# JeongsooP/RGB-no-more

Hardware: AMD Instinct MI355X
Metric: images/sec JPEG-Ti DCT 512x512 train step (higher is better)
Workload: dtype bf16

## Files before the change

### rgb-no-more_amd/csrc/internal.h

```cpp
#pragma once
#include <hip/hip_runtime.h>

constexpr int RGBNM_TN_MAX_SPLIT = 128;
struct RgbnmTnJob {
  const void* dY; const void* X; float* part; float* bpart;
  int ldy, ldx, M, No, Ki;
  float* dW; float* db; int perm_heads, accumulate;
  int smax;
};
int rgbnm_launch_tn_pipe_group(const RgbnmTnJob* jobs, int n, int* S_out, hipStream_t st, int* direct_out = nullptr);
void rgbnm_tn_defer_begin();
void rgbnm_tn_defer_begin_n(int max_jobs);
int rgbnm_tn_defer_flush(hipStream_t st);
int rgbnm_launch_tn_pipe(const void* dY, int ldy, const void* X, int ldx, float* part, float* bpart, int M, int No,
                         int Ki, int* S_out, hipStream_t st, int smax = 0);

int rgbnm_launch_attn2_fwd(const void* qkv, void* out, float* lse, int B, int N, int heads, float scale,
                           hipStream_t st);
int rgbnm_launch_attn2_bwd(const void* qkv, const void* out, const void* dout, const float* lse, void* dqkv, int B,
                           int N, int heads, float scale, hipStream_t st);

enum { TR_NT = 1, TR_TN = 2, TR_ATTN_FWD = 3, TR_ATTN_BWD = 4, TR_CHAIN_FWD = 5, TR_CHAIN_BWD = 6, TR_AUG = 7, TR_EMBED = 8, TR_OPT = 9 };
int rgbnm_launch_nt_wres(int epi, const void* A, int lda, const void* W, int ldw, void* C, int ldc, const float* bias,
                         const void* R, int ldr, void* C2, int ldc2, int M, int N, int K, hipStream_t st);
int rgbnm_launch_nt_kpipe(int epi, const void* A, int lda, const void* W, int ldw, void* C, int ldc, const float* bias,
                          const void* R, int ldr, void* C2, int ldc2, int M, int N, int K, hipStream_t st);
int rgbnm_launch_nt_kpipe_res_ln(const void* A, int lda, const void* W, int ldw, const float* bias, const void* R,
                                 int ldr, void* x, int ldc, const float* gamma, const float* beta, void* y, int ldy,
                                 float* mean, float* rstd, float eps, int M, int N, int K, hipStream_t st);
int rgbnm_launch_mlp_fwd(const void* X, int ldx, const void* W1, const float* b1, const void* W2, const float* b2,
                         const void* R, int ldr, void* G, void* GP, int ldg, void* Y, int ldy, const float* gamma,
                         const float* beta, void* Y2, int ldy2, float* mean, float* rstd, float eps, int M, int E, int H,
                         hipStream_t st);
int rgbnm_launch_nt_small(int epi, const void* A, int lda, const void* W, int ldw, void* C, int ldc, const float* bias,
                          const void* R, int ldr, int c_f32, int M, int N, int K, hipStream_t st);
int rgbnm_launch_mlp_bwd(const void* DY, int lddy, const void* W2T, const void* W1T, const void* GP, int ldg, void* DU, int ldu,
                         const void* X, int ldx, const float* gamma, const float* mean, const float* rstd, void* DX, int lddx,
                         float* part, int* npanels_out, int M, int E, int H, hipStream_t st);
int rgbnm_launch_nt_kpipe_lnbwd(const void* A, int lda, const void* W, int ldw, const void* X, int ldx,
                                const float* gamma, const float* mean, const float* rstd, const void* dres, int ldr,
                                void* dx, int ldc, float* part, int* npanels_out, int M, int N, int K, hipStream_t st);
struct RgbnmReduceJob {
  const float* part; long long stride; float* out;
  int n, S, cols, perm_heads, accumulate, epw;
};
bool rgbnm_reduce_defer_active();
void rgbnm_reduce_defer_begin();
int rgbnm_reduce_defer_flush(hipStream_t st);
int rgbnm_reduce_submit(const RgbnmReduceJob& job, hipStream_t st);
int rgbnm_trace_begin(int tag, double flops, double bytes, hipStream_t st);
void rgbnm_trace_end(int slot, hipStream_t st);
```

### rgb-no-more_amd/csrc/layernorm.hip

```cpp
#include "common.h"
#include "../../include/rgbnm.h"
#include "internal.h"

namespace {


template <int LPR>
__device__ __forceinline__ float row_sum(float v) {
  if constexpr (LPR == 16) return group16_sum(v);
  else if constexpr (LPR == 32) return group16_sum(v + __shfl_xor(v, 16, 64));
  else return wave_sum(v);
}

template <typename T, int NV, int LPR = 16>
__global__ __launch_bounds__(256) void ln_fwd_kernel(const T* __restrict__ x, const float* __restrict__ gamma,
                                                     const float* __restrict__ beta, T* __restrict__ y,
                                                     float* __restrict__ mean, float* __restrict__ rstd, int M,
                                                     float eps) {
  constexpr int E = NV * LPR * 4, G = 256 / LPR;
  const int l16 = threadIdx.x & (LPR - 1), grp = threadIdx.x / LPR;
  f32x4 gm[NV], bt[NV];
#pragma unroll
  for (int v = 0; v < NV; ++v) {
    gm[v] = *reinterpret_cast<const f32x4*>(gamma + (v * LPR + l16) * 4);
    bt[v] = *reinterpret_cast<const f32x4*>(beta + (v * LPR + l16) * 4);
  }
  for (int row = blockIdx.x * G + grp; row < M; row += gridDim.x * G) {
#pragma clang fp contract(off)
    f32x4 xv[NV];
    float s = 0.f;
#pragma unroll
    for (int v = 0; v < NV; ++v) {
      xv[v] = load4<T>(x + (size_t)row * E + (v * LPR + l16) * 4);
      s += xv[v][0] + xv[v][1] + xv[v][2] + xv[v][3];
    }
// ... 91 lines not shown
      float a = 0.f;
#pragma unroll
      for (int r = 0; r < G; ++r) a += red[r][e];
      part[((size_t)blockIdx.x * 2 + pass) * E + e] = a;
    }
  }
}

int submit_ln_reduce(const float* part, float* dgamma, float* dbeta, int nblk, int E, int accumulate, hipStream_t st) {
  RgbnmReduceJob j;
  j.part = part; j.stride = 2LL * E; j.out = dgamma; j.n = E; j.S = nblk; j.cols = 1; j.perm_heads = 0;
  j.accumulate = accumulate; j.epw = 8;
  const bool own = !rgbnm_reduce_defer_active();
  if (own) rgbnm_reduce_defer_begin();
  int rc = rgbnm_reduce_submit(j, st);
  if (rc == RGBNM_OK) {
    j.part = part + E; j.out = dbeta;
    rc = rgbnm_reduce_submit(j, st);
  }
  if (own) {
    const int rf = rgbnm_reduce_defer_flush(st);
    if (rc == RGBNM_OK) rc = rf;
  }
  return rc;
}

template <typename T, int NV, int LPR = 16>
__global__ __launch_bounds__(256) void pool_fwd_kernel(const T* __restrict__ x, const float* __restrict__ gamma,
                                                       const float* __restrict__ beta, T* __restrict__ pooled,
                                                       float* __restrict__ mean, float* __restrict__ rstd, int N,
                                                       float eps) {
  constexpr int E = NV * LPR * 4, G = 256 / LPR;
  __shared__ float red[G][E + 4];
  const int b = blockIdx.x;
  const int l16 = threadIdx.x & (LPR - 1), grp = threadIdx.x / LPR;
  f32x4 acc[NV];
#pragma unroll
  for (int v = 0; v < NV; ++v) acc[v] = (f32x4){0.f, 0.f, 0.f, 0.f};
  constexpr int UNR = 8;
  for (int t0 = grp; t0 < N; t0 += UNR * G) {
    f32x4 xa[UNR][NV];
#pragma unroll
    for (int u = 0; u < UNR; ++u) {
      const int tt = min(t0 + u * G, N - 1);
#pragma unroll
      for (int v = 0; v < NV; ++v) xa[u][v] = load4<T>(x + ((size_t)b * N + tt) * E + (v * LPR + l16) * 4);
    }
#pragma unroll
    for (int u = 0; u < UNR; ++u) {
    const int t = t0 + u * G;
    if (t >= N) break;
    const size_t row = (size_t)b * N + t;
    f32x4 xv[NV];
    float s = 0.f;
#pragma unroll
    for (int v = 0; v < NV; ++v) {
      xv[v] = xa[u][v];
      s += xv[v][0] + xv[v][1] + xv[v][2] + xv[v][3];
    }
    const float mu = row_sum<LPR>(s) * (1.f / E);
    float q = 0.f;
#pragma unroll
    for (int v = 0; v < NV; ++v)
#pragma unroll
      for (int i = 0; i < 4; ++i) {
        const float d = xv[v][i] - mu;
        q += d * d;
      }
    const float rs = rsqrtf(row_sum<LPR>(q) * (1.f / E) + eps);
#pragma unroll
    for (int v = 0; v < NV; ++v)
#pragma unroll
      for (int i = 0; i < 4; ++i) acc[v][i] += (xv[v][i] - mu) * rs;
    if (l16 == 0) {
      mean[row] = mu;
      rstd[row] = rs;
    }
    }
  }
#pragma unroll
  for (int v = 0; v < NV; ++v)
#pragma unroll
    for (int i = 0; i < 4; ++i) red[grp][(v * LPR + l16) * 4 + i] = acc[v][i];
  __syncthreads();
  for (int e = threadIdx.x; e < E; e += 256) {
    float a = 0.f;
#pragma unroll
    for (int r = 0; r < G; ++r) a += red[r][e];
    pooled[(size_t)b * E + e] = from_f32<T>(a * (1.f / N) * gamma[e] + beta[e]);
  }
}

template <typename T, int NV, int LPR = 16>
__global__ __launch_bounds__(256) void pool_bwd_kernel(const T* __restrict__ dpooled, const T* __restrict__ x,
                                                       const float* __restrict__ gamma, const float* __restrict__ mean,
                                                       const float* __restrict__ rstd, T* __restrict__ dx,
                                                       float* __restrict__ part, int N) {
  constexpr int E = NV * LPR * 4, G = 256 / LPR;
  __shared__ float red[G][E + 4];
  const int b = blockIdx.x;
  const int l16 = threadIdx.x & (LPR - 1), grp = threadIdx.x / LPR;
  const float invN = 1.f / N;
  f32x4 gm[NV], dv[NV], dg[NV];
#pragma unroll
  for (int v = 0; v < NV; ++v) {
    gm[v] = *reinterpret_cast<const f32x4*>(gamma + (v * LPR + l16) * 4);
    dv[v] = load4<T>(dpooled + (size_t)b * E + (v * LPR + l16) * 4);
#pragma unroll
    for (int i = 0; i < 4; ++i) dv[v][i] *= invN;
    dg[v] = (f32x4){0.f, 0.f, 0.f, 0.f};
  }
  constexpr int UNR = 4;
  for (int t0 = grp; t0 < N; t0 += UNR * G) {
    f32x4 xa[UNR][NV];
    float mua[UNR], rsa[UNR];
#pragma unroll
    for (int u = 0; u < UNR; ++u) {
      const int tt = min(t0 + u * G, N - 1);
      mua[u] = mean[(size_t)b * N + tt];
      rsa[u] = rstd[(size_t)b * N + tt];
#pragma unroll
      for (int v = 0; v < NV; ++v) xa[u][v] = load4<T>(x + ((size_t)b * N + tt) * E + (v * LPR + l16) * 4);
    }
#pragma unroll
    for (int u = 0; u < UNR; ++u) {
    const int t = t0 + u * G;
    if (t >= N) break;
    const size_t row = (size_t)b * N + t;
    const float mu = mua[u], rs = rsa[u];
    f32x4 xh[NV], gv[NV];
    float s1 = 0.f, s2 = 0.f;
#pragma unroll
    for (int v = 0; v < NV; ++v) {
      const f32x4 xv = xa[u][v];
#pragma unroll
      for (int i = 0; i < 4; ++i) {
        xh[v][i] = (xv[i] - mu) * rs;
        gv[v][i] = dv[v][i] * gm[v][i];
        s1 += gv[v][i];
        s2 += gv[v][i] * xh[v][i];
        dg[v][i] += dv[v][i] * xh[v][i];
      }
    }
    const float c1 = row_sum<LPR>(s1) * (1.f / E), c2 = row_sum<LPR>(s2) * (1.f / E);
#pragma unroll
    for (int v = 0; v < NV; ++v) {
      f32x4 o;
#pragma unroll
      for (int i = 0; i < 4; ++i) o[i] = rs * (gv[v][i] - c1 - xh[v][i] * c2);
      store4<T>(dx + row * E + (v * LPR + l16) * 4, o);
    }
    }
  }
#pragma unroll
  for (int v = 0; v < NV; ++v)
#pragma unroll
    for (int i = 0; i < 4; ++i) red[grp][(v * LPR + l16) * 4 + i] = dg[v][i];
  __syncthreads();
  for (int e = threadIdx.x; e < E; e += 256) {
    float a = 0.f;
#pragma unroll
    for (int r = 0; r < G; ++r) a += red[r][e];
    part[((size_t)b * 2 + 0) * E + e] = a;
    part[((size_t)b * 2 + 1) * E + e] = to_f32(dpooled[(size_t)b * E + e]);
  }
}

constexpr int LN_BWD_BLOCKS = 2048;

template <typename T>
int ln_fwd_t(const void* x, const float* g, const float* b, void* y, float* mean, float* rstd, int M, int E, float eps,
             hipStream_t st) {
  const int grid = min(cdiv(M, E <= 384 ? 16 : 4), 4096);
  if (E == 192) hipLaunchKernelGGL((ln_fwd_kernel<T, 3>), dim3(grid), dim3(256), 0, st, (const T*)x, g, b, (T*)y, mean, rstd, M, eps);
  else if (E == 384) hipLaunchKernelGGL((ln_fwd_kernel<T, 6>), dim3(grid), dim3(256), 0, st, (const T*)x, g, b, (T*)y, mean, rstd, M, eps);
  else if (E == 512) hipLaunchKernelGGL((ln_fwd_kernel<T, 2, 64>), dim3(grid), dim3(256), 0, st, (const T*)x, g, b, (T*)y, mean, rstd, M, eps);
  else if (E == 768) hipLaunchKernelGGL((ln_fwd_kernel<T, 3, 64>), dim3(grid), dim3(256), 0, st, (const T*)x, g, b, (T*)y, mean, rstd, M, eps);
  else if (E == 1024) hipLaunchKernelGGL((ln_fwd_kernel<T, 4, 64>), dim3(grid), dim3(256), 0, st, (const T*)x, g, b, (T*)y, mean, rstd, M, eps);
  else return RGBNM_EINVAL;
  LAUNCH_CHECK();
  return RGBNM_OK;
}

template <typename T>
int ln_bwd_t(const void* dy, const void* x, const float* g, const float* mean, const float* rstd, const void* dres,
             void* dx, float* dgamma, float* dbeta, int M, int E, int accumulate, float* ws, hipStream_t st) {
  const int P = cdiv(M, E == 192 ? 16 : E == 384 ? 8 : 4), grid = cdiv(P, cdiv(P, LN_BWD_BLOCKS));
  if (E == 192) hipLaunchKernelGGL((ln_bwd_kernel<T, 3>), dim3(grid), dim3(256), 0, st, (const T*)dy, (const T*)x, g, mean, rstd, (const T*)dres, (T*)dx, ws, M);
  else if (E == 384) hipLaunchKernelGGL((ln_bwd_kernel<T, 3, 32>), dim3(grid), dim3(256), 0, st, (const T*)dy, (const T*)x, g, mean, rstd, (const T*)dres, (T*)dx, ws, M);
  else if (E == 512) hipLaunchKernelGGL((ln_bwd_kernel<T, 2, 64>), dim3(grid), dim3(256), 0, st, (const T*)dy, (const T*)x, g, mean, rstd, (const T*)dres, (T*)dx, ws, M);
  else if (E == 768) hipLaunchKernelGGL((ln_bwd_kernel<T, 3, 64>), dim3(grid), dim3(256), 0, st, (const T*)dy, (const T*)x, g, mean, rstd, (const T*)dres, (T*)dx, ws, M);
  else if (E == 1024) hipLaunchKernelGGL((ln_bwd_kernel<T, 4, 64>), dim3(grid), dim3(256), 0, st, (const T*)dy, (const T*)x, g, mean, rstd, (const T*)dres, (T*)dx, ws, M);
  else return RGBNM_EINVAL;
  LAUNCH_CHECK();
  return submit_ln_reduce(ws, dgamma, dbeta, grid, E, accumulate, st);
}

}
// ... 86 lines not shown
```

### rgb-no-more_amd/csrc/vit.hip

```cpp
#include "common.h"
#include "../../include/rgbnm.h"

#define TRY(x)                 \
  do {                         \
    int rc__ = (x);            \
    if (rc__ != 0) return rc__; \
  } while (0)

static inline size_t max_sz(size_t a, size_t b) { return a > b ? a : b; }

#include <string.h>
#include <atomic>
#include <mutex>
#include <vector>
#include "internal.h"
namespace {
std::mutex g_trace_mu;
struct TraceRec { hipEvent_t a, b; int tag; double flops, bytes; };
std::vector<TraceRec> g_recs;
std::vector<hipEvent_t> g_event_pool;
hipEvent_t take_event() {
  if (!g_event_pool.empty()) { hipEvent_t e = g_event_pool.back(); g_event_pool.pop_back(); return e; }
  hipEvent_t e = nullptr;
  if (hipEventCreate(&e) != hipSuccess) return nullptr;
  return e;
}
struct Opt { const char* name; std::atomic<int> value; };
Opt g_opts[] = {{"nt_staged", 1}, {"tn_tr", 1}, {"tn_pipe", 1}, {"attn_v2", 1}, {"nt_wres", 1}, {"nt_kpipe", 1}, {"attn_persist", 1}, {"ln_fuse", 1}, {"tn_group", 2}, {"trace", 0}, {"tn_wgs", 512}, {"mlp_fuse", 1}, {"nt_cold", 0}, {"mlp_bwd", 1}, {"nt_small", 1}, {"mlp_dmast", 1}, {"gelu_table", 1}, {"ln_rows", 1}, {"kp8", 1}, {"win_xcd", 1}, {"kp_persist", 1}, {"fwd_chain", 1}, {"bwd_chain", 1}, {"tn_direct", 1}, {"tn_pack", 1}, {"tn_wide", 1}};
}

int rgbnm_trace_begin(int tag, double flops, double bytes, hipStream_t st) {
  int mask = 0;
  for (auto& o : g_opts) if (!strcmp(o.name, "trace")) mask = o.value.load(std::memory_order_relaxed);
  if (!((mask >> tag) & 1)) return -1;
  std::lock_guard<std::mutex> lk(g_trace_mu);
  TraceRec r;
  r.a = take_event();
  r.b = take_event();
  if (!r.a || !r.b) return -1;
  r.tag = tag; r.flops = flops; r.bytes = bytes;
  (void)hipEventRecord(r.a, st);
  g_recs.push_back(r);
  return (int)g_recs.size() - 1;
}
void rgbnm_trace_end(int slot, hipStream_t st) {
  if (slot < 0) return;
  std::lock_guard<std::mutex> lk(g_trace_mu);
  if (slot >= 0 && slot < (int)g_recs.size()) (void)hipEventRecord(g_recs[slot].b, st);
}

extern "C" {

int rgbnm_abi_version(void) { return RGBNM_ABI_VERSION; }

int rgbnm_set_option(const char* name, int value) {
  for (auto& o : g_opts)
    if (name && !strcmp(o.name, name)) { o.value.store(value, std::memory_order_relaxed); return RGBNM_OK; }
  return RGBNM_EINVAL;
}
int rgbnm_get_option(const char* name) {
  for (auto& o : g_opts)
// ... 283 lines not shown
    }
    if (pe_dx0) TRY(rgbnm_gemm_tn(dt, pe_dx0, E, pe_feat, 384, pe_dw, pe_db, M, E, 384, 0, 0, pe_ws, pe_ws_bytes, st));
    if (group) { tn_open = false; TRY(rgbnm_tn_defer_flush((hipStream_t)st)); }
    for (int i = 0; i < n; ++i) {
      RgbnmReduceJob j;
      j.stride = 2LL * E; j.n = E; j.S = c->B; j.cols = 1; j.perm_heads = 0; j.accumulate = 0; j.epw = 8;
      j.part = part2[i]; j.out = g[i]->dln2_g;
      TRY(rgbnm_reduce_submit(j, (hipStream_t)st));
      j.part = part2[i] + E; j.out = g[i]->dln2_b;
      TRY(rgbnm_reduce_submit(j, (hipStream_t)st));
      j.part = part1[i]; j.out = g[i]->dln1_g;
      TRY(rgbnm_reduce_submit(j, (hipStream_t)st));
      j.part = part1[i] + E; j.out = g[i]->dln1_b;
      TRY(rgbnm_reduce_submit(j, (hipStream_t)st));
    }
    return RGBNM_OK;
  }();
  const int rt = tn_open ? rgbnm_tn_defer_flush((hipStream_t)st) : RGBNM_OK;
  const int rf = rgbnm_reduce_defer_flush((hipStream_t)st);
  return rc != RGBNM_OK ? rc : (rt != RGBNM_OK ? rt : rf);
}

int rgbnm_vit_block_bwd_dw(const rgbnm_vit_cfg* c, const rgbnm_block_acts* a, const rgbnm_block_grads* g,
                           const rgbnm_block_scratch* s, const void* dy, const float* part2, const float* part1, void* st) {
  return rgbnm_vit_blocks_bwd_dw(c, 1, &a, &g, &s, &dy, &part2, &part1, st);
}

int rgbnm_patch_embed_fwd_mix(const rgbnm_vit_cfg* c, int in_dtype, const void* y, const void* cbcr, const float* lam_dev,
                              const float* conv16, const void* wpe, const float* bpe, const float* pos, void* feat, void* x0, int Hb,
                              int Wb, void* st) {
  if (!c) return RGBNM_EINVAL;
  const int M = c->B * c->N;
  if ((Hb / 2) * (Wb / 2) != c->N) return RGBNM_EINVAL;
  TRY(rgbnm_subblock_embed_mix(in_dtype, c->dtype, y, cbcr, lam_dev, conv16, feat, c->B, Hb, Wb, 0, st));
  TRY(rgbnm_gemm_nt(c->dtype, RGBNM_EPI_POS, feat, 384, wpe, 384, x0, c->E, bpe, 0, 0, 0, 0, pos, c->N, M, c->E, 384,
                    0, st));
  return RGBNM_OK;
}

int rgbnm_patch_embed_fwd(const rgbnm_vit_cfg* c, int in_dtype, const void* y, const void* cbcr, const float* conv16,
                          const void* wpe, const float* bpe, const float* pos, void* feat, void* x0, int Hb, int Wb,
                          void* st) {
  return rgbnm_patch_embed_fwd_mix(c, in_dtype, y, cbcr, nullptr, conv16, wpe, bpe, pos, feat, x0, Hb, Wb, st);
}

int rgbnm_patch_embed_bwd(const rgbnm_vit_cfg* c, const void* dx0, const void* feat, float* dwpe, float* dbpe,
                          void* ws, size_t ws_bytes, void* st) {
  if (!c) return RGBNM_EINVAL;
  return rgbnm_gemm_tn(c->dtype, dx0, c->E, feat, 384, dwpe, dbpe, c->B * c->N, c->E, 384, 0, 0, ws, ws_bytes, st);
}

int rgbnm_head_fwd(const rgbnm_vit_cfg* c, const rgbnm_head_params* p, const rgbnm_head_acts* a, void* st) {
  if (!c || !p || !a) return RGBNM_EINVAL;
  const int dt = c->dtype, E = c->E, C = p->n_classes;
  TRY(rgbnm_head_pool_fwd(dt, a->x, p->ln_g, p->ln_b, a->pooled, a->mean, a->rstd, c->B, c->N, E, c->ln_eps, st));
  TRY(rgbnm_gemm_nt(dt, RGBNM_EPI_TANH, a->pooled, E, p->w1, E, a->h1, E, p->b1, 0, 0, 0, 0, 0, 0, c->B, E, E, 0, st));
  TRY(rgbnm_gemm_nt(dt, RGBNM_EPI_NONE, a->h1, E, p->w2, E, a->logits, C, p->b2, 0, 0, 0, 0, 0, 0, c->B, C, E, 1, st));
  return RGBNM_OK;
}

size_t rgbnm_head_bwd_workspace(const rgbnm_vit_cfg* c, int n_classes) {
  if (!c) return 0;
  return ((rgbnm_gemm_tn_workspace(c->B, n_classes, c->E) + 255) & ~(size_t)255) + ((rgbnm_gemm_tn_workspace(c->B, c->E, c->E) + 255) & ~(size_t)255) +
         (size_t)c->B * 2 * c->E * sizeof(float);
}

int rgbnm_head_bwd(const rgbnm_vit_cfg* c, const rgbnm_head_params* p, const rgbnm_head_acts* a,
                   const rgbnm_head_grads* g, const void* dlogits, void* da, void* dpooled, void* dx, void* ws,
                   size_t ws_bytes, void* st) {
  if (!c || !p || !a || !g || !dlogits || !da || !dpooled || !dx) return RGBNM_EINVAL;
  const int dt = c->dtype, E = c->E, C = p->n_classes, B = c->B;
  const size_t s1 = (rgbnm_gemm_tn_workspace(B, C, E) + 255) & ~(size_t)255, s2 = (rgbnm_gemm_tn_workspace(B, E, E) + 255) & ~(size_t)255;
  const size_t s3 = (size_t)B * 2 * E * sizeof(float);
  const bool apart = ws_bytes >= s1 + s2 + s3;
  char* w1 = (char*)ws;
  char* w2 = apart ? w1 + s1 : w1;
  char* w3 = apart ? w2 + s2 : w1;
  const size_t b1 = apart ? s1 : ws_bytes, b2 = apart ? s2 : ws_bytes, b3 = apart ? ws_bytes - s1 - s2 : ws_bytes;
  const bool grouped = apart && rgbnm_get_option("tn_group") != 0;
  if (grouped) rgbnm_tn_defer_begin();
  const int rc = [&]() -> int {
    TRY(rgbnm_gemm_tn(dt, dlogits, C, a->h1, E, g->dw2, g->db2, B, C, E, 0, 0, w1, b1, st));
    TRY(rgbnm_gemm_nt(dt, RGBNM_EPI_DTANH, dlogits, C, p->w2_t, C, da, E, 0, a->h1, E, 0, 0, 0, 0, B, E, C, 0, st));
    TRY(rgbnm_gemm_tn(dt, da, E, a->pooled, E, g->dw1, g->db1, B, E, E, 0, 0, w2, b2, st));
    return RGBNM_OK;
  }();
  const int rt = grouped ? rgbnm_tn_defer_flush((hipStream_t)st) : RGBNM_OK;
  if (rc != RGBNM_OK) return rc;
  if (rt != RGBNM_OK) return rt;
  TRY(rgbnm_gemm_nt(dt, RGBNM_EPI_NONE, da, E, p->w1_t, E, dpooled, E, 0, 0, 0, 0, 0, 0, 0, B, E, E, 0, st));
  TRY(rgbnm_head_pool_bwd(dt, dpooled, a->x, p->ln_g, a->mean, a->rstd, dx, g->dln_g, g->dln_b, B, c->N, E, 0, w3, b3, st));
  return RGBNM_OK;
}

}
```

Measured before the change: 65690.

## Fuse patch-embed and classifier head fwd/bwd into single per-image kernels

Adds a fused patch-embed kernel that combines the subblock embedding mix with the projection GEMM, bias and positional add. It also adds fused head forward (pool+LN, tanh matvec, logits) and backward (dlogits matvec, dtanh, dpooled matvec, pool LN backward) kernels, one block per image. The aim is to remove several small kernel launches and intermediate global round-trips for small-M GEMMs. The trade-off is that the per-image blocks do matvecs with low MMA utilisation and limited parallelism, and the new paths are gated on bf16 with E=192.

```diff
diff --git a/rgb-no-more_amd/csrc/head_fused.hip b/rgb-no-more_amd/csrc/head_fused.hip
--- /dev/null
+++ b/rgb-no-more_amd/csrc/head_fused.hip
@@ -0,0 +1,200 @@
+#include "common.h"
+#include "internal.h"
+#include "pool_rows.h"
+
+namespace {
+
+constexpr int E = 192, NV = 3, LPR = 16, G = 256 / LPR;
+constexpr int CH = 1024;
+
+struct HeadFwd {
+  const bf16* x; const float* ln_g; const float* ln_b; const bf16* w1; const float* b1; const bf16* w2; const float* b2;
+  bf16* pooled; float* mean; float* rstd; bf16* h1; float* logits;
+  int N, C; float eps;
+};
+struct HeadBwd {
+  const bf16* dlogits; const bf16* w2t; const bf16* w1t; const bf16* h1; const bf16* x; const float* ln_g;
+  const float* mean; const float* rstd;
+  bf16* da; bf16* dpooled; bf16* dx; float* part;
+  int N, C;
+};
+
+__device__ __forceinline__ bf16x8 kfrag(const bf16* row, int k, int K) {
+  const bf16x8 zero = {0, 0, 0, 0, 0, 0, 0, 0};
+  return k < K ? *reinterpret_cast<const bf16x8*>(row + k) : zero;
+}
+
+__device__ __forceinline__ void matvec192(const bf16* a, const bf16* __restrict__ W, int ldw, int K, float (*part)[CH], int w,
+                                          int lane) {
+  const int l31 = lane & 31, g = lane >> 5;
+  const int ksteps = (K + 15) / 16, per = (ksteps + 3) / 4;
+  const int s0 = w * per, s1 = min(s0 + per, ksteps);
+  f32x16 acc[6];
+#pragma unroll
+  for (int t = 0; t < 6; ++t)
+#pragma unroll
+    for (int r = 0; r < 16; ++r) acc[t][r] = 0.f;
+  const bf16* wrow = W + (size_t)l31 * ldw;
+  for (int s = s0; s < s1; s += 4) {
+    Frag<bf16> fa[4], fw[4][6];
+#pragma unroll
+    for (int u = 0; u < 4; ++u) {
+      const int k = 16 * (s + u < s1 ? s + u : s1 - 1) + 8 * g;
+      fa[u].v = kfrag(a, k, K);
+#pragma unroll
+      for (int t = 0; t < 6; ++t) fw[u][t].v = kfrag(wrow + (size_t)(32 * t) * ldw, k, K);
+    }
+#pragma unroll
+    for (int u = 0; u < 4; ++u)
+      if (s + u < s1) {
+#pragma unroll
+        for (int t = 0; t < 6; ++t) mma(acc[t], fw[u][t], fa[u]);
+      }
+  }
+  if (l31 == 0) {
+#pragma unroll
+    for (int t = 0; t < 6; ++t)
+#pragma unroll
+      for (int q = 0; q < 4; ++q) {
+        const f32x4 v = {acc[t][4 * q + 0], acc[t][4 * q + 1], acc[t][4 * q + 2], acc[t][4 * q + 3]};
+        *reinterpret_cast<f32x4*>(&part[w][32 * t + 8 * q + 4 * g]) = v;
+      }
+  }
+}
+
+__device__ __forceinline__ float sum4(float (*part)[CH], int n) {
+  float v = part[0][n];
+#pragma unroll
+  for (int k = 1; k < 4; ++k) v += part[k][n];
+  return v;
+}
+
+__global__ __launch_bounds__(256) void head_fwd_fused_kernel(HeadFwd p) {
+  __shared__ float red[G][E + 4];
+  __shared__ __attribute__((aligned(16))) float part[4][CH];
+  __shared__ __attribute__((aligned(16))) bf16 sp[E], sh[E];
+  const int b = blockIdx.x, tid = threadIdx.x, lane = tid & 63;
+  const int w = __builtin_amdgcn_readfirstlane(tid >> 6);
+  const int l31 = lane & 31, g = lane >> 5;
+  pool_fwd_image<bf16, NV, LPR>(p.x, p.ln_g, p.ln_b, p.pooled, p.mean, p.rstd, p.N, p.eps, b, red, sp);
+  __syncthreads();
+  matvec192(sp, p.w1, E, E, part, w, lane);
+  __syncthreads();
+  if (tid < E) {
+    float v = sum4(part, tid);
+    v += p.b1[tid];
+    float x = (float)(bf16)v;
+    x = tanhf(x);
+    const bf16 o = (bf16)x;
+    p.h1[(size_t)b * E + tid] = o;
+    sh[tid] = o;
+  }
+  __syncthreads();
+  Frag<bf16> fa[3];
+#pragma unroll
+  for (int u = 0; u < 3; ++u) fa[u].v = *reinterpret_cast<const bf16x8*>(&sh[16 * (3 * w + u) + 8 * g]);
+  for (int c0 = 0; c0 < p.C; c0 += CH) {
+    const int cn = min(CH, p.C - c0);
+    for (int n0 = 0; n0 < cn; n0 += 8 * 32) {
+      Frag<bf16> fw[8][3];
+#pragma unroll
+      for (int t = 0; t < 8; ++t) {
+        const bf16* wrow = p.w2 + (size_t)min(c0 + n0 + 32 * t + l31, p.C - 1) * E + 16 * 3 * w + 8 * g;
+#pragma unroll
+        for (int u = 0; u < 3; ++u) fw[t][u].v = *reinterpret_cast<const bf16x8*>(wrow + 16 * u);
+      }
+#pragma unroll
+      for (int t = 0; t < 8; ++t) {
+        f32x16 acc;
+#pragma unroll
+        for (int r = 0; r < 16; ++r) acc[r] = 0.f;
+#pragma unroll
+        for (int u = 0; u < 3; ++u) mma(acc, fw[t][u], fa[u]);
+        if (l31 == 0) {
+#pragma unroll
+          for (int q = 0; q < 4; ++q) {
+            const int n = n0 + 32 * t + 8 * q + 4 * g;
+            const f32x4 v = {acc[4 * q + 0], acc[4 * q + 1], acc[4 * q + 2], acc[4 * q + 3]};
+            if (n < cn) *reinterpret_cast<f32x4*>(&part[w][n]) = v;
+          }
+        }
+      }
+    }
+    __syncthreads();
+    for (int n = tid; n < cn; n += 256) {
+      float v = sum4(part, n);
+      if (p.b2) v += p.b2[c0 + n];
+      p.logits[(size_t)b * p.C + c0 + n] = v;
+    }
+    __syncthreads();
+  }
+}
+
+__global__ __launch_bounds__(256) void head_bwd_fused_kernel(HeadBwd p) {
+  __shared__ float red[G][E + 4];
+  __shared__ __attribute__((aligned(16))) float part[4][CH];
+  __shared__ __attribute__((aligned(16))) bf16 sda[E], sdp[E];
+  const int b = blockIdx.x, tid = threadIdx.x, lane = tid & 63;
+  const int w = __builtin_amdgcn_readfirstlane(tid >> 6);
+  matvec192(p.dlogits + (size_t)b * p.C, p.w2t, p.C, p.C, part, w, lane);
+  __syncthreads();
+  if (tid < E) {
+    const float v = sum4(part, tid);
+    float x = (float)(bf16)v;
+    const float h = (float)p.h1[(size_t)b * E + tid];
+    x *= (1.f - h * h);
+    const bf16 o = (bf16)x;
+    p.da[(size_t)b * E + tid] = o;
+    sda[tid] = o;
+  }
+  __syncthreads();
+  matvec192(sda, p.w1t, E, E, part, w, lane);
+  __syncthreads();
+  if (tid < E) {
+    const float v = sum4(part, tid);
+    const float x = (float)(bf16)v;
+    const bf16 o = (bf16)x;
+    p.dpooled[(size_t)b * E + tid] = o;
+    sdp[tid] = o;
+  }
+  __syncthreads();
+  pool_bwd_image<bf16, NV, LPR>(sdp, p.x, p.ln_g, p.mean, p.rstd, p.dx, p.part, p.N, b, red);
+}
+
+}
+
+int rgbnm_launch_head_fwd_fused(const void* x, const float* ln_g, const float* ln_b, const void* w1, const float* b1, const void* w2,
+                                const float* b2, void* pooled, float* mean, float* rstd, void* h1, float* logits, int B, int N, int C,
+                                float eps, hipStream_t st) {
+  if (!x || !ln_g || !ln_b || !w1 || !b1 || !w2 || !pooled || !mean || !rstd || !h1 || !logits || B <= 0 || N <= 0) return RGBNM_EINVAL;
+  if (B > 512 || C <= 0 || C % 8) return 1;
+  HeadFwd p;
+  p.x = (const bf16*)x; p.ln_g = ln_g; p.ln_b = ln_b; p.w1 = (const bf16*)w1; p.b1 = b1; p.w2 = (const bf16*)w2; p.b2 = b2;
+  p.pooled = (bf16*)pooled; p.mean = mean; p.rstd = rstd; p.h1 = (bf16*)h1; p.logits = logits; p.N = N; p.C = C; p.eps = eps;
+  const double Bd = B;
+  const int slot = rgbnm_trace_begin(TR_NT, 2.0 * Bd * E * E + 2.0 * Bd * C * E,
+                                     (Bd * E + (double)E * E) * 2.0 + Bd * E * 2.0 + (Bd * E + (double)C * E) * 2.0 + Bd * C * 4.0, st);
+  hipLaunchKernelGGL(head_fwd_fused_kernel, dim3(B), dim3(256), 0, st, p);
+  rgbnm_trace_end(slot, st);
+  LAUNCH_CHECK();
+  return RGBNM_OK;
+}
+
+int rgbnm_launch_head_bwd_fused(const void* dlogits, const void* w2t, const void* w1t, const void* h1, const void* x, const float* ln_g,
+                                const float* mean, const float* rstd, void* da, void* dpooled, void* dx, float* part, int B, int N,
+                                int C, hipStream_t st) {
+  if (!dlogits || !w2t || !w1t || !h1 || !x || !ln_g || !mean || !rstd || !da || !dpooled || !dx || !part || B <= 0 || N <= 0)
+    return RGBNM_EINVAL;
+  if (B > 512 || C <= 0 || C % 8) return 1;
+  HeadBwd p;
+  p.dlogits = (const bf16*)dlogits; p.w2t = (const bf16*)w2t; p.w1t = (const bf16*)w1t; p.h1 = (const bf16*)h1; p.x = (const bf16*)x;
+  p.ln_g = ln_g; p.mean = mean; p.rstd = rstd; p.da = (bf16*)da; p.dpooled = (bf16*)dpooled; p.dx = (bf16*)dx; p.part = part;
+  p.N = N; p.C = C;
+  const double Bd = B;
+  const int slot = rgbnm_trace_begin(TR_NT, 2.0 * Bd * E * C + 2.0 * Bd * E * E,
+                                     (Bd * C + (double)E * C) * 2.0 + Bd * E * 4.0 + (Bd * E + (double)E * E) * 2.0 + Bd * E * 2.0, st);
+  hipLaunchKernelGGL(head_bwd_fused_kernel, dim3(B), dim3(256), 0, st, p);
+  rgbnm_trace_end(slot, st);
+  LAUNCH_CHECK();
+  return RGBNM_OK;
+}
diff --git a/rgb-no-more_amd/csrc/internal.h b/rgb-no-more_amd/csrc/internal.h
--- a/rgb-no-more_amd/csrc/internal.h
+++ b/rgb-no-more_amd/csrc/internal.h
@@ -34,6 +34,15 @@
                          hipStream_t st);
 int rgbnm_launch_nt_small(int epi, const void* A, int lda, const void* W, int ldw, void* C, int ldc, const float* bias,
                           const void* R, int ldr, int c_f32, int M, int N, int K, hipStream_t st);
+int rgbnm_launch_patch_embed_fused(int in_dtype, const void* y, const void* cbcr, const float* lam_dev, const float* conv16,
+                                   const void* wpe, const float* bpe, const float* pos, void* feat, void* x0, int B, int Hb, int Wb,
+                                   hipStream_t st);
+int rgbnm_launch_head_fwd_fused(const void* x, const float* ln_g, const float* ln_b, const void* w1, const float* b1, const void* w2,
+                                const float* b2, void* pooled, float* mean, float* rstd, void* h1, float* logits, int B, int N, int C,
+                                float eps, hipStream_t st);
+int rgbnm_launch_head_bwd_fused(const void* dlogits, const void* w2t, const void* w1t, const void* h1, const void* x, const float* ln_g,
+                                const float* mean, const float* rstd, void* da, void* dpooled, void* dx, float* part, int B, int N,
+                                int C, hipStream_t st);
 int rgbnm_launch_mlp_bwd(const void* DY, int lddy, const void* W2T, const void* W1T, const void* GP, int ldg, void* DU, int ldu,
                          const void* X, int ldx, const float* gamma, const float* mean, const float* rstd, void* DX, int lddx,
                          float* part, int* npanels_out, int M, int E, int H, hipStream_t st);
diff --git a/rgb-no-more_amd/csrc/layernorm.hip b/rgb-no-more_amd/csrc/layernorm.hip
--- a/rgb-no-more_amd/csrc/layernorm.hip
+++ b/rgb-no-more_amd/csrc/layernorm.hip
@@ -1,6 +1,7 @@
 #include "common.h"
 #include "../../include/rgbnm.h"
 #include "internal.h"
+#include "pool_rows.h"
 
 namespace {
 
@@ -158,63 +159,7 @@
                                                        float eps) {
   constexpr int E = NV * LPR * 4, G = 256 / LPR;
   __shared__ float red[G][E + 4];
-  const int b = blockIdx.x;
-  const int l16 = threadIdx.x & (LPR - 1), grp = threadIdx.x / LPR;
-  f32x4 acc[NV];
-#pragma unroll
-  for (int v = 0; v < NV; ++v) acc[v] = (f32x4){0.f, 0.f, 0.f, 0.f};
-  constexpr int UNR = 8;
-  for (int t0 = grp; t0 < N; t0 += UNR * G) {
-    f32x4 xa[UNR][NV];
-#pragma unroll
-    for (int u = 0; u < UNR; ++u) {
-      const int tt = min(t0 + u * G, N - 1);
-#pragma unroll
-      for (int v = 0; v < NV; ++v) xa[u][v] = load4<T>(x + ((size_t)b * N + tt) * E + (v * LPR + l16) * 4);
-    }
-#pragma unroll
-    for (int u = 0; u < UNR; ++u) {
-    const int t = t0 + u * G;
-    if (t >= N) break;
-    const size_t row = (size_t)b * N + t;
-    f32x4 xv[NV];
-    float s = 0.f;
-#pragma unroll
-    for (int v = 0; v < NV; ++v) {
-      xv[v] = xa[u][v];
-      s += xv[v][0] + xv[v][1] + xv[v][2] + xv[v][3];
-    }
-    const float mu = row_sum<LPR>(s) * (1.f / E);
-    float q = 0.f;
-#pragma unroll
-    for (int v = 0; v < NV; ++v)
-#pragma unroll
-      for (int i = 0; i < 4; ++i) {
-        const float d = xv[v][i] - mu;
-        q += d * d;
-      }
-    const float rs = rsqrtf(row_sum<LPR>(q) * (1.f / E) + eps);
-#pragma unroll
-    for (int v = 0; v < NV; ++v)
-#pragma unroll
-      for (int i = 0; i < 4; ++i) acc[v][i] += (xv[v][i] - mu) * rs;
-    if (l16 == 0) {
-      mean[row] = mu;
-      rstd[row] = rs;
-    }
-    }
-  }
-#pragma unroll
-  for (int v = 0; v < NV; ++v)
-#pragma unroll
-    for (int i = 0; i < 4; ++i) red[grp][(v * LPR + l16) * 4 + i] = acc[v][i];
-  __syncthreads();
-  for (int e = threadIdx.x; e < E; e += 256) {
-    float a = 0.f;
-#pragma unroll
-    for (int r = 0; r < G; ++r) a += red[r][e];
-    pooled[(size_t)b * E + e] = from_f32<T>(a * (1.f / N) * gamma[e] + beta[e]);
-  }
+  pool_fwd_image<T, NV, LPR>(x, gamma, beta, pooled, mean, rstd, N, eps, blockIdx.x, red, nullptr);
 }
 
 template <typename T, int NV, int LPR = 16>
@@ -224,72 +169,7 @@
                                                        float* __restrict__ part, int N) {
   constexpr int E = NV * LPR * 4, G = 256 / LPR;
   __shared__ float red[G][E + 4];
-  const int b = blockIdx.x;
-  const int l16 = threadIdx.x & (LPR - 1), grp = threadIdx.x / LPR;
-  const float invN = 1.f / N;
-  f32x4 gm[NV], dv[NV], dg[NV];
-#pragma unroll
-  for (int v = 0; v < NV; ++v) {
-    gm[v] = *reinterpret_cast<const f32x4*>(gamma + (v * LPR + l16) * 4);
-    dv[v] = load4<T>(dpooled + (size_t)b * E + (v * LPR + l16) * 4);
-#pragma unroll
-    for (int i = 0; i < 4; ++i) dv[v][i] *= invN;
-    dg[v] = (f32x4){0.f, 0.f, 0.f, 0.f};
-  }
-  constexpr int UNR = 4;
-  for (int t0 = grp; t0 < N; t0 += UNR * G) {
-    f32x4 xa[UNR][NV];
-    float mua[UNR], rsa[UNR];
-#pragma unroll
-    for (int u = 0; u < UNR; ++u) {
-      const int tt = min(t0 + u * G, N - 1);
-      mua[u] = mean[(size_t)b * N + tt];
-      rsa[u] = rstd[(size_t)b * N + tt];
-#pragma unroll
-      for (int v = 0; v < NV; ++v) xa[u][v] = load4<T>(x + ((size_t)b * N + tt) * E + (v * LPR + l16) * 4);
-    }
-#pragma unroll
-    for (int u = 0; u < UNR; ++u) {
-    const int t = t0 + u * G;
-    if (t >= N) break;
-    const size_t row = (size_t)b * N + t;
-    const float mu = mua[u], rs = rsa[u];
-    f32x4 xh[NV], gv[NV];
-    float s1 = 0.f, s2 = 0.f;
-#pragma unroll
-    for (int v = 0; v < NV; ++v) {
-      const f32x4 xv = xa[u][v];
-#pragma unroll
-      for (int i = 0; i < 4; ++i) {
-        xh[v][i] = (xv[i] - mu) * rs;
-        gv[v][i] = dv[v][i] * gm[v][i];
-        s1 += gv[v][i];
-        s2 += gv[v][i] * xh[v][i];
-        dg[v][i] += dv[v][i] * xh[v][i];
-      }
-    }
-    const float c1 = row_sum<LPR>(s1) * (1.f / E), c2 = row_sum<LPR>(s2) * (1.f / E);
-#pragma unroll
-    for (int v = 0; v < NV; ++v) {
-      f32x4 o;
-#pragma unroll
-      for (int i = 0; i < 4; ++i) o[i] = rs * (gv[v][i] - c1 - xh[v][i] * c2);
-      store4<T>(dx + row * E + (v * LPR + l16) * 4, o);
-    }
-    }
-  }
-#pragma unroll
-  for (int v = 0; v < NV; ++v)
-#pragma unroll
-    for (int i = 0; i < 4; ++i) red[grp][(v * LPR + l16) * 4 + i] = dg[v][i];
-  __syncthreads();
-  for (int e = threadIdx.x; e < E; e += 256) {
-    float a = 0.f;
-#pragma unroll
-    for (int r = 0; r < G; ++r) a += red[r][e];
-    part[((size_t)b * 2 + 0) * E + e] = a;
-    part[((size_t)b * 2 + 1) * E + e] = to_f32(dpooled[(size_t)b * E + e]);
-  }
+  pool_bwd_image<T, NV, LPR>(dpooled + (size_t)blockIdx.x * E, x, gamma, mean, rstd, dx, part, N, blockIdx.x, red);
 }
 
 constexpr int LN_BWD_BLOCKS = 2048;
diff --git a/rgb-no-more_amd/csrc/patch_embed_fused.hip b/rgb-no-more_amd/csrc/patch_embed_fused.hip
--- /dev/null
+++ b/rgb-no-more_amd/csrc/patch_embed_fused.hip
@@ -0,0 +1,192 @@
+#include "common.h"
+#include "internal.h"
+
+namespace {
+
+constexpr int PR = 98;
+constexpr int KF = 384, EO = 192;
+constexpr int PITCH = KF * 2 + 16;
+constexpr int XS_BYTES = 4 * 16 * 17 * 4;
+constexpr int SMEM = PR * PITCH + XS_BYTES;
+constexpr int PF = 6;
+
+struct PeFused {
+  const void* y; const void* cbcr; const float* A; const float* lam; const bf16* W; const float* bias; const float* pos;
+  bf16* feat; bf16* x0;
+  int B, Hb, Wb, nh, ps;
+};
+
+__device__ __forceinline__ float mix2(float a, float c, float l0, float l1) { return fmaf(c, l1, a * l0); }
+
+template <typename TI>
+__global__ __launch_bounds__(256) __attribute__((amdgpu_waves_per_eu(2, 2))) void patch_embed_fused_kernel(PeFused p) {
+  extern __shared__ __attribute__((aligned(16))) unsigned char smem[];
+  unsigned char* As = smem;
+  float (*Xs)[16][17] = reinterpret_cast<float (*)[16][17]>(smem + PR * PITCH);
+  const int tid = threadIdx.x, lane = tid & 63;
+  const int w = __builtin_amdgcn_readfirstlane(tid >> 6);
+  const int img = blockIdx.x / p.nh, panel = blockIdx.x % p.nh;
+  const int ph_n = p.Hb / 2, pw_n = p.Wb / 2, npos = ph_n * pw_n;
+  const int t0 = panel * p.ps, nr = min(p.ps, npos - t0);
+  if (nr <= 0) return;
+  bf16* featp = p.feat + ((size_t)img * npos + t0) * KF;
+  {
+    const TI* y = reinterpret_cast<const TI*>(p.y);
+    const TI* cbcr = reinterpret_cast<const TI*>(p.cbcr);
+    const int g = lane >> 4, c = lane & 15;
+    float a1[4], a2[4];
+#pragma unroll
+    for (int kk = 0; kk < 4; ++kk) {
+      a1[kk] = p.A[c * 16 + 4 * kk + g];
+      a2[kk] = p.A[c * 16 + 4 * g + kk];
+    }
+    const int pdh = lane >> 5, pdw = (lane >> 4) & 1, l16 = lane & 15;
+    const int p1 = l16 >> 1, p2 = (l16 & 1) * 4;
+    const int e0 = lane * 2, cc = e0 >> 6, k = e0 & 63;
+    const bool mixed = p.lam != nullptr;
+    const float l0 = mixed ? p.lam[0] : 1.f, l1 = mixed ? p.lam[1] : 0.f;
+    const size_t ypi = (size_t)p.Hb * p.Wb * 64, cpi = (size_t)2 * npos * 64;
+    const int pb = img == 0 ? p.B - 1 : img - 1;
+    struct alignas(2 * sizeof(TI)) TI2 { TI a, b; };
+    struct Raw { typename Vec4<TI>::type v; TI2 c; };
+    auto fetch = [&](int pos, int b, Raw& r) {
+      const int ph = pos / pw_n, pw = pos % pw_n;
+      r.v = *reinterpret_cast<const typename Vec4<TI>::type*>(y + b * ypi + ((size_t)(2 * ph + pdh) * p.Wb + 2 * pw + pdw) * 64 + l16 * 4);
+      r.c = *reinterpret_cast<const TI2*>(cbcr + b * cpi + (((size_t)cc * ph_n + ph) * pw_n + pw) * 64 + k);
+    };
+    int fi = w;
+    Raw rq[PF] = {}, sq[PF] = {};
+    auto fetch_next = [&](Raw& r, Raw& s) {
+      if (fi < nr) {
+        fetch(t0 + fi, img, r);
+        if (mixed) fetch(t0 + fi, pb, s);
+      }
+      fi += 4;
+    };
+#pragma unroll
+    for (int u = 0; u < PF; ++u) fetch_next(rq[u], sq[u]);
+    for (int i = w; i < nr; i += 4) {
+      const Raw cur = rq[0], prev = sq[0];
+#pragma unroll
+      for (int u = 0; u + 1 < PF; ++u) {
+        rq[u] = rq[u + 1];
+        sq[u] = sq[u + 1];
+      }
+      fetch_next(rq[PF - 1], sq[PF - 1]);
+      f32x4 v = {to_f32(cur.v[0]), to_f32(cur.v[1]), to_f32(cur.v[2]), to_f32(cur.v[3])};
+      float c0 = to_f32(cur.c.a), c1 = to_f32(cur.c.b);
+      if (mixed) {
+#pragma unroll
+        for (int e = 0; e < 4; ++e) v[e] = to_f32(from_f32<TI>(mix2(v[e], to_f32(prev.v[e]), l0, l1)));
+        c0 = to_f32(from_f32<TI>(mix2(c0, to_f32(prev.c.a), l0, l1)));
+        c1 = to_f32(from_f32<TI>(mix2(c1, to_f32(prev.c.b), l0, l1)));
+      }
+#pragma unroll
+      for (int e = 0; e < 4; ++e) Xs[w][8 * pdh + p1][8 * pdw + p2 + e] = v[e];
+      asm volatile("s_waitcnt lgkmcnt(0)" ::: "memory");
+      f32x4 t = {0.f, 0.f, 0.f, 0.f};
+#pragma unroll
+      for (int kk = 0; kk < 4; ++kk) t = __builtin_amdgcn_mfma_f32_16x16x4f32(Xs[w][4 * kk + g][c], a1[kk], t, 0, 0, 0);
+      asm volatile("s_waitcnt lgkmcnt(0)" ::: "memory");
+      f32x4 z = {0.f, 0.f, 0.f, 0.f};
+#pragma unroll
+      for (int kk = 0; kk < 4; ++kk) z = __builtin_amdgcn_mfma_f32_16x16x4f32(a2[kk], t[kk], z, 0, 0, 0);
+      const bf16x4 zb = {from_f32<bf16>(z[0]), from_f32<bf16>(z[1]), from_f32<bf16>(z[2]), from_f32<bf16>(z[3])};
+      struct alignas(4) Pair { bf16 a, b; };
+      Pair pr;
+      pr.a = from_f32<bf16>(c0);
+      pr.b = from_f32<bf16>(c1);
+      bf16* dst = featp + (size_t)i * KF;
+      *reinterpret_cast<bf16x4*>(dst + c * 16 + 4 * g) = zb;
+      *reinterpret_cast<Pair*>(dst + 256 + e0) = pr;
+      bf16* lrow = reinterpret_cast<bf16*>(As + i * PITCH);
+      *reinterpret_cast<bf16x4*>(lrow + c * 16 + 4 * g) = zb;
+      *reinterpret_cast<Pair*>(lrow + 256 + e0) = pr;
+    }
+  }
+  __syncthreads();
+  if (32 * w >= nr) return;
+  const int l31 = lane & 31, g = lane >> 5;
+  const int tl = min(32 * w + l31, nr - 1);
+  const unsigned char* arow = As + tl * PITCH + 16 * g;
+  const bf16* wrow = p.W + (size_t)l31 * KF + 8 * g;
+  f32x16 acc[6];
+#pragma unroll
+  for (int t = 0; t < 6; ++t)
+#pragma unroll
+    for (int r = 0; r < 16; ++r) acc[t][r] = 0.f;
+  for (int ks = 0; ks < KF / 16; ks += 4) {
+    Frag<bf16> fa[4], fw[4][6];
+#pragma unroll
+    for (int u = 0; u < 4; ++u) {
+      fa[u].v = *reinterpret_cast<const bf16x8*>(arow + (ks + u) * 32);
+#pragma unroll
+      for (int t = 0; t < 6; ++t) fw[u][t].v = *reinterpret_cast<const bf16x8*>(wrow + (size_t)(32 * t) * KF + 16 * (ks + u));
+    }
+#pragma unroll
+    for (int u = 0; u < 4; ++u)
+#pragma unroll
+      for (int t = 0; t < 6; ++t) mma(acc[t], fw[u][t], fa[u]);
+  }
+  asm volatile("s_waitcnt lgkmcnt(0)" ::: "memory");
+  const float* posr = p.pos + (size_t)(t0 + tl) * EO;
+  const bool valid = 32 * w + l31 < nr;
+  bf16* srow = reinterpret_cast<bf16*>(As + (32 * w + l31) * PITCH);
+#pragma unroll
+  for (int t = 0; t < 6; ++t)
+#pragma unroll
+    for (int q = 0; q < 4; ++q) {
+      const int nl = 32 * t + 8 * q + 4 * g;
+      f32x4 v = {acc[t][4 * q + 0], acc[t][4 * q + 1], acc[t][4 * q + 2], acc[t][4 * q + 3]};
+      if (p.bias) {
+        const f32x4 bv = *reinterpret_cast<const f32x4*>(p.bias + nl);
+        v += bv;
+      }
+      const f32x4 pv = *reinterpret_cast<const f32x4*>(posr + nl);
+      v += pv;
+      if (valid) store4<bf16>(srow + nl, v);
+    }
+  asm volatile("s_waitcnt lgkmcnt(0)" ::: "memory");
+  bf16* x0p = p.x0 + ((size_t)img * npos + t0 + 32 * w) * EO;
+#pragma unroll
+  for (int it = 0; it < 32 * (EO / 8) / 64; ++it) {
+    const int idx = it * 64 + lane, row = idx / (EO / 8), vec = idx % (EO / 8);
+    if (32 * w + row < nr) {
+      const bf16x8 cv = *reinterpret_cast<const bf16x8*>(As + (32 * w + row) * PITCH + vec * 16);
+      *reinterpret_cast<bf16x8*>(x0p + (size_t)row * EO + vec * 8) = cv;
+    }
+  }
+}
+
+}
+
+int rgbnm_launch_patch_embed_fused(int in_dtype, const void* y, const void* cbcr, const float* lam_dev, const float* conv16,
+                                   const void* wpe, const float* bpe, const float* pos, void* feat, void* x0, int B, int Hb, int Wb,
+                                   hipStream_t st) {
+  if (!y || !cbcr || !conv16 || !wpe || !pos || !feat || !x0 || B <= 0 || Hb <= 0 || Wb <= 0 || (Hb & 1) || (Wb & 1)) return RGBNM_EINVAL;
+  if (in_dtype != DT_F32 && in_dtype != DT_BF16) return 1;
+  const int npos = (Hb / 2) * (Wb / 2);
+  const long long npatch = (long long)B * npos;
+  if (npatch * KF >= (1LL << 31)) return RGBNM_EINVAL;
+  PeFused p;
+  p.y = y; p.cbcr = cbcr; p.A = conv16; p.lam = lam_dev; p.W = (const bf16*)wpe; p.bias = bpe; p.pos = pos;
+  p.feat = (bf16*)feat; p.x0 = (bf16*)x0; p.B = B; p.Hb = Hb; p.Wb = Wb;
+  p.nh = cdiv(npos, PR);
+  p.ps = cdiv(npos, p.nh);
+  static DevOnce attr;
+  if (attr.need()) {
+    if (hipFuncSetAttribute((const void*)patch_embed_fused_kernel<float>, hipFuncAttributeMaxDynamicSharedMemorySize, SMEM) != hipSuccess ||
+        hipFuncSetAttribute((const void*)patch_embed_fused_kernel<bf16>, hipFuncAttributeMaxDynamicSharedMemorySize, SMEM) != hipSuccess)
+      return RGBNM_ELAUNCH;
+    attr.done();
+  }
+  const double np = (double)npatch;
+  const int slot = rgbnm_trace_begin(TR_EMBED, 4.0 * np * 16 * 16 * 16 + 2.0 * np * EO * KF,
+                                     np * KF * ((in_dtype == DT_F32 ? 4.0 : 2.0) + 2.0) + (np * KF + (double)EO * KF) * 2.0 + np * EO * 2.0, st);
+  const dim3 grid((unsigned)(B * p.nh)), blk(256);
+  if (in_dtype == DT_F32) hipLaunchKernelGGL(patch_embed_fused_kernel<float>, grid, blk, SMEM, st, p);
+  else hipLaunchKernelGGL(patch_embed_fused_kernel<bf16>, grid, blk, SMEM, st, p);
+  rgbnm_trace_end(slot, st);
+  LAUNCH_CHECK();
+  return RGBNM_OK;
+}
diff --git a/rgb-no-more_amd/csrc/pool_rows.h b/rgb-no-more_amd/csrc/pool_rows.h
--- /dev/null
+++ b/rgb-no-more_amd/csrc/pool_rows.h
@@ -0,0 +1,148 @@
+#pragma once
+#include "common.h"
+
+template <int LPR>
+__device__ __forceinline__ float pool_row_sum(float v) {
+  if constexpr (LPR == 16) return group16_sum(v);
+  else if constexpr (LPR == 32) return group16_sum(v + __shfl_xor(v, 16, 64));
+  else return wave_sum(v);
+}
+
+template <typename T, int NV, int LPR>
+__device__ __forceinline__ void pool_fwd_image(const T* __restrict__ x, const float* __restrict__ gamma,
+                                               const float* __restrict__ beta, T* __restrict__ pooled,
+                                               float* __restrict__ mean, float* __restrict__ rstd, int N, float eps, int b,
+                                               float (*red)[NV * LPR * 4 + 4], T* pooled_lds) {
+  constexpr int E = NV * LPR * 4, G = 256 / LPR;
+  const int l16 = threadIdx.x & (LPR - 1), grp = threadIdx.x / LPR;
+  f32x4 acc[NV];
+#pragma unroll
+  for (int v = 0; v < NV; ++v) acc[v] = (f32x4){0.f, 0.f, 0.f, 0.f};
+  constexpr int UNR = 8;
+  for (int t0 = grp; t0 < N; t0 += UNR * G) {
+    f32x4 xa[UNR][NV];
+#pragma unroll
+    for (int u = 0; u < UNR; ++u) {
+      const int tt = min(t0 + u * G, N - 1);
+#pragma unroll
+      for (int v = 0; v < NV; ++v) xa[u][v] = load4<T>(x + ((size_t)b * N + tt) * E + (v * LPR + l16) * 4);
+    }
+#pragma unroll
+    for (int u = 0; u < UNR; ++u) {
+    const int t = t0 + u * G;
+    if (t >= N) break;
+    const size_t row = (size_t)b * N + t;
+    f32x4 xv[NV];
+    float s = 0.f;
+#pragma unroll
+    for (int v = 0; v < NV; ++v) {
+      xv[v] = xa[u][v];
+      s += xv[v][0] + xv[v][1] + xv[v][2] + xv[v][3];
+    }
+    const float mu = pool_row_sum<LPR>(s) * (1.f / E);
+    float q = 0.f;
+#pragma unroll
+    for (int v = 0; v < NV; ++v)
+#pragma unroll
+      for (int i = 0; i < 4; ++i) {
+        const float d = xv[v][i] - mu;
+        q += d * d;
+      }
+    const float rs = rsqrtf(pool_row_sum<LPR>(q) * (1.f / E) + eps);
+#pragma unroll
+    for (int v = 0; v < NV; ++v)
+#pragma unroll
+      for (int i = 0; i < 4; ++i) acc[v][i] += (xv[v][i] - mu) * rs;
+    if (l16 == 0) {
+      mean[row] = mu;
+      rstd[row] = rs;
+    }
+    }
+  }
+#pragma unroll
+  for (int v = 0; v < NV; ++v)
+#pragma unroll
+    for (int i = 0; i < 4; ++i) red[grp][(v * LPR + l16) * 4 + i] = acc[v][i];
+  __syncthreads();
+  for (int e = threadIdx.x; e < E; e += 256) {
+    float a = 0.f;
+#pragma unroll
+    for (int r = 0; r < G; ++r) a += red[r][e];
+    const T o = from_f32<T>(a * (1.f / N) * gamma[e] + beta[e]);
+    pooled[(size_t)b * E + e] = o;
+    if (pooled_lds) pooled_lds[e] = o;
+  }
+}
+
+template <typename T, int NV, int LPR>
+__device__ __forceinline__ void pool_bwd_image(const T* dprow, const T* __restrict__ x, const float* __restrict__ gamma,
+                                               const float* __restrict__ mean, const float* __restrict__ rstd,
+                                               T* __restrict__ dx, float* __restrict__ part, int N, int b,
+                                               float (*red)[NV * LPR * 4 + 4]) {
+  constexpr int E = NV * LPR * 4, G = 256 / LPR;
+  const int l16 = threadIdx.x & (LPR - 1), grp = threadIdx.x / LPR;
+  const float invN = 1.f / N;
+  f32x4 gm[NV], dv[NV], dg[NV];
+#pragma unroll
+  for (int v = 0; v < NV; ++v) {
+    gm[v] = *reinterpret_cast<const f32x4*>(gamma + (v * LPR + l16) * 4);
+    dv[v] = load4<T>(dprow + (v * LPR + l16) * 4);
+#pragma unroll
+    for (int i = 0; i < 4; ++i) dv[v][i] *= invN;
+    dg[v] = (f32x4){0.f, 0.f, 0.f, 0.f};
+  }
+  constexpr int UNR = 4;
+  for (int t0 = grp; t0 < N; t0 += UNR * G) {
+    f32x4 xa[UNR][NV];
+    float mua[UNR], rsa[UNR];
+#pragma unroll
+    for (int u = 0; u < UNR; ++u) {
+      const int tt = min(t0 + u * G, N - 1);
+      mua[u] = mean[(size_t)b * N + tt];
+      rsa[u] = rstd[(size_t)b * N + tt];
+#pragma unroll
+      for (int v = 0; v < NV; ++v) xa[u][v] = load4<T>(x + ((size_t)b * N + tt) * E + (v * LPR + l16) * 4);
+    }
+#pragma unroll
+    for (int u = 0; u < UNR; ++u) {
+    const int t = t0 + u * G;
+    if (t >= N) break;
+    const size_t row = (size_t)b * N + t;
+    const float mu = mua[u], rs = rsa[u];
+    f32x4 xh[NV], gv[NV];
+    float s1 = 0.f, s2 = 0.f;
+#pragma unroll
+    for (int v = 0; v < NV; ++v) {
+      const f32x4 xv = xa[u][v];
+#pragma unroll
+      for (int i = 0; i < 4; ++i) {
+        xh[v][i] = (xv[i] - mu) * rs;
+        gv[v][i] = dv[v][i] * gm[v][i];
+        s1 += gv[v][i];
+        s2 += gv[v][i] * xh[v][i];
+        dg[v][i] += dv[v][i] * xh[v][i];
+      }
+    }
+    const float c1 = pool_row_sum<LPR>(s1) * (1.f / E), c2 = pool_row_sum<LPR>(s2) * (1.f / E);
+#pragma unroll
+    for (int v = 0; v < NV; ++v) {
+      f32x4 o;
+#pragma unroll
+      for (int i = 0; i < 4; ++i) o[i] = rs * (gv[v][i] - c1 - xh[v][i] * c2);
+      store4<T>(dx + row * E + (v * LPR + l16) * 4, o);
+    }
+    }
+  }
+#pragma unroll
+  for (int v = 0; v < NV; ++v)
+#pragma unroll
+    for (int i = 0; i < 4; ++i) red[grp][(v * LPR + l16) * 4 + i] = dg[v][i];
+  __syncthreads();
+  for (int e = threadIdx.x; e < E; e += 256) {
+    float a = 0.f;
+#pragma unroll
+    for (int r = 0; r < G; ++r) a += red[r][e];
+    part[((size_t)b * 2 + 0) * E + e] = a;
+    part[((size_t)b * 2 + 1) * E + e] = to_f32(dprow[e]);
+  }
+}
diff --git a/rgb-no-more_amd/csrc/vit.hip b/rgb-no-more_amd/csrc/vit.hip
--- a/rgb-no-more_amd/csrc/vit.hip
+++ b/rgb-no-more_amd/csrc/vit.hip
@@ -26,7 +26,7 @@
   return e;
 }
 struct Opt { const char* name; std::atomic<int> value; };
-Opt g_opts[] = {{"nt_staged", 1}, {"tn_tr", 1}, {"tn_pipe", 1}, {"attn_v2", 1}, {"nt_wres", 1}, {"nt_kpipe", 1}, {"attn_persist", 1}, {"ln_fuse", 1}, {"tn_group", 2}, {"trace", 0}, {"tn_wgs", 512}, {"mlp_fuse", 1}, {"nt_cold", 0}, {"mlp_bwd", 1}, {"nt_small", 1}, {"mlp_dmast", 1}, {"gelu_table", 1}, {"ln_rows", 1}, {"kp8", 1}, {"win_xcd", 1}, {"kp_persist", 1}, {"fwd_chain", 1}, {"bwd_chain", 1}, {"tn_direct", 1}, {"tn_pack", 1}, {"tn_wide", 1}};
+Opt g_opts[] = {{"nt_staged", 1}, {"tn_tr", 1}, {"tn_pipe", 1}, {"attn_v2", 1}, {"nt_wres", 1}, {"nt_kpipe", 1}, {"attn_persist", 1}, {"ln_fuse", 1}, {"tn_group", 2}, {"trace", 0}, {"tn_wgs", 512}, {"mlp_fuse", 1}, {"nt_cold", 0}, {"mlp_bwd", 1}, {"nt_small", 1}, {"mlp_dmast", 1}, {"gelu_table", 1}, {"ln_rows", 1}, {"kp8", 1}, {"win_xcd", 1}, {"kp_persist", 1}, {"fwd_chain", 1}, {"bwd_chain", 1}, {"tn_direct", 1}, {"tn_pack", 1}, {"tn_wide", 1}, {"pe_fuse", 1}, {"head_fuse", 1}};
 }
 
 int rgbnm_trace_begin(int tag, double flops, double bytes, hipStream_t st) {
@@ -376,6 +376,11 @@
   if (!c) return RGBNM_EINVAL;
   const int M = c->B * c->N;
   if ((Hb / 2) * (Wb / 2) != c->N) return RGBNM_EINVAL;
+  if (c->dtype == RGBNM_DT_BF16 && c->E == 192 && (in_dtype == RGBNM_DT_F32 || in_dtype == RGBNM_DT_BF16) && rgbnm_get_option("pe_fuse")) {
+    const int rc = rgbnm_launch_patch_embed_fused(in_dtype, y, cbcr, lam_dev, conv16, wpe, bpe, pos, feat, x0, c->B, Hb, Wb,
+                                                  (hipStream_t)st);
+    if (rc <= 0) return rc;
+  }
   TRY(rgbnm_subblock_embed_mix(in_dtype, c->dtype, y, cbcr, lam_dev, conv16, feat, c->B, Hb, Wb, 0, st));
   TRY(rgbnm_gemm_nt(c->dtype, RGBNM_EPI_POS, feat, 384, wpe, 384, x0, c->E, bpe, 0, 0, 0, 0, pos, c->N, M, c->E, 384,
                     0, st));
@@ -394,9 +399,19 @@
   return rgbnm_gemm_tn(c->dtype, dx0, c->E, feat, 384, dwpe, dbpe, c->B * c->N, c->E, 384, 0, 0, ws, ws_bytes, st);
 }
 
+static bool head_fused_ok(const rgbnm_vit_cfg* c, int C) {
+  return c->dtype == RGBNM_DT_BF16 && c->E == 192 && c->B <= 512 && C > 0 && C % 8 == 0 && rgbnm_get_option("head_fuse") &&
+         rgbnm_get_option("nt_small");
+}
+
 int rgbnm_head_fwd(const rgbnm_vit_cfg* c, const rgbnm_head_params* p, const rgbnm_head_acts* a, void* st) {
   if (!c || !p || !a) return RGBNM_EINVAL;
   const int dt = c->dtype, E = c->E, C = p->n_classes;
+  if (head_fused_ok(c, C)) {
+    const int rc = rgbnm_launch_head_fwd_fused(a->x, p->ln_g, p->ln_b, p->w1, p->b1, p->w2, p->b2, a->pooled, a->mean, a->rstd, a->h1,
+                                               a->logits, c->B, c->N, C, c->ln_eps, (hipStream_t)st);
+    if (rc <= 0) return rc;
+  }
   TRY(rgbnm_head_pool_fwd(dt, a->x, p->ln_g, p->ln_b, a->pooled, a->mean, a->rstd, c->B, c->N, E, c->ln_eps, st));
   TRY(rgbnm_gemm_nt(dt, RGBNM_EPI_TANH, a->pooled, E, p->w1, E, a->h1, E, p->b1, 0, 0, 0, 0, 0, 0, c->B, E, E, 0, st));
   TRY(rgbnm_gemm_nt(dt, RGBNM_EPI_NONE, a->h1, E, p->w2, E, a->logits, C, p->b2, 0, 0, 0, 0, 0, 0, c->B, C, E, 1, st));
@@ -422,16 +437,44 @@
   char* w3 = apart ? w2 + s2 : w1;
   const size_t b1 = apart ? s1 : ws_bytes, b2 = apart ? s2 : ws_bytes, b3 = apart ? ws_bytes - s1 - s2 : ws_bytes;
   const bool grouped = apart && rgbnm_get_option("tn_group") != 0;
+  bool fused = head_fused_ok(c, C);
+  if (fused && (!a->x || !p->ln_g || !a->mean || !a->rstd || !g->dln_g || !g->dln_b || !ws)) return RGBNM_EINVAL;
+  if (fused && b3 < s3) return RGBNM_EWORKSPACE;
   if (grouped) rgbnm_tn_defer_begin();
   const int rc = [&]() -> int {
     TRY(rgbnm_gemm_tn(dt, dlogits, C, a->h1, E, g->dw2, g->db2, B, C, E, 0, 0, w1, b1, st));
-    TRY(rgbnm_gemm_nt(dt, RGBNM_EPI_DTANH, dlogits, C, p->w2_t, C, da, E, 0, a->h1, E, 0, 0, 0, 0, B, E, C, 0, st));
+    if (fused) {
+      const int rf = rgbnm_launch_head_bwd_fused(dlogits, p->w2_t, p->w1_t, a->h1, a->x, p->ln_g, a->mean, a->rstd, da, dpooled, dx,
+                                                 (float*)w3, B, c->N, C, (hipStream_t)st);
+      if (rf < 0) return rf;
+      fused = rf == 0;
+    }
+    if (fused) {
+      RgbnmReduceJob j;
+      j.part = (const float*)w3; j.stride = 2LL * E; j.out = g->dln_g; j.n = E; j.S = B; j.cols = 1; j.perm_heads = 0;
+      j.accumulate = 0; j.epw = 8;
+      const bool own = !rgbnm_reduce_defer_active();
+      if (own) rgbnm_reduce_defer_begin();
+      int rr = rgbnm_reduce_submit(j, (hipStream_t)st);
+      if (rr == RGBNM_OK) {
+        j.part = (const float*)w3 + E; j.out = g->dln_b;
+        rr = rgbnm_reduce_submit(j, (hipStream_t)st);
+      }
+      if (own) {
+        const int rl = rgbnm_reduce_defer_flush((hipStream_t)st);
+        if (rr == RGBNM_OK) rr = rl;
+      }
+      TRY(rr);
+    } else {
+      TRY(rgbnm_gemm_nt(dt, RGBNM_EPI_DTANH, dlogits, C, p->w2_t, C, da, E, 0, a->h1, E, 0, 0, 0, 0, B, E, C, 0, st));
+    }
     TRY(rgbnm_gemm_tn(dt, da, E, a->pooled, E, g->dw1, g->db1, B, E, E, 0, 0, w2, b2, st));
     return RGBNM_OK;
   }();
   const int rt = grouped ? rgbnm_tn_defer_flush((hipStream_t)st) : RGBNM_OK;
   if (rc != RGBNM_OK) return rc;
   if (rt != RGBNM_OK) return rt;
+  if (fused) return RGBNM_OK;
   TRY(rgbnm_gemm_nt(dt, RGBNM_EPI_NONE, da, E, p->w1_t, E, dpooled, E, 0, 0, 0, 0, 0, 0, 0, B, E, E, 0, st));
   TRY(rgbnm_head_pool_bwd(dt, dpooled, a->x, p->ln_g, a->mean, a->rstd, dx, g->dln_g, g->dln_b, B, c->N, E, 0, w3, b3, st));
   return RGBNM_OK;
```

New measurement: 64790. -1.4%, worse.
